# Acelogic/Retrieval-based-Voice-Conversion-MLX

Measured on AMD Instinct MI355X. Metric: audio-sec/sec (realtime factor) RVCv2 48kHz pipeline, higher is better.
Workload: dtype fp32-accurate (two-plane fp16 MFMA split); 1 GPU; C2: full RVCv2 48kHz pipeline, one 13.5 s utterance per step per GPU; samples_16k=216100, x_pad=1, f0_method=rmvpe, parallelism=dp1

## Files before the change

### retrieval-based-voice-conversion-mlx_amd/csrc/resblock_fused.hip

```cpp
#include <algorithm>

#include "conv_common.h"
#include "split_bf16.h"

namespace rvcx {

namespace {

using namespace splitbf16;

constexpr int RB_THREADS = 256;
constexpr int RB_MAXH1 = 30;

__host__ __device__ constexpr int rb_pi(int j) { return (j & 3) | (((j >> 3) & 1) << 2) | (((j >> 2) & 1) << 3); }

enum RbFmt : int { RB_BF16X3 = 0, RB_F16X2 = 1, RB_F16X1 = 2 };
__host__ __device__ constexpr int rb_planes(int fmt) { return fmt == RB_BF16X3 ? 3 : (fmt == RB_F16X2 ? 2 : 1); }

template <int C, int FMT = RB_BF16X3>
struct RbGeo {
  static constexpr int NCH = C / 16;
  static constexpr int NP = rb_planes(FMT);
  static constexpr int ROW = NCH * NP * 32 + 16;
};
// ... 383 lines not shown
#pragma unroll
      for (int q = 0; q < NQ; ++q) {
        w1r[st][q] = *reinterpret_cast<const f16x8_*>(p1 + (size_t)st * 2 * QS + q * QS);
        w2r[st][q] = *reinterpret_cast<const f16x8_*>(p2 + (size_t)st * 2 * QS + q * QS);
      }
  }
  if (tid < 4 * C) {
    const int which = tid / C, c = tid % C;
    const float* inv1 = reinterpret_cast<const float*>(static_cast<const char*>(a.w1s) + NST * 2 * QS);
    const float* inv2 = reinterpret_cast<const float*>(static_cast<const char*>(a.w2s) + NST * 2 * QS);
    prm[tid] = which == 0 ? a.b1[c] : which == 1 ? inv1[c] : which == 2 ? a.b2[c] : inv2[c];
  }

  f32x4 xv[XITER];
  unsigned xok = 0u;
  auto load_x = [&](int tl) __attribute__((always_inline)) {
    const int bb = tl / ntiles, tb = (tl - bb * ntiles) * TT - 1 - h1;
    const float* Xb = a.x + (long long)bb * a.x_bs;
    xok = 0u;
#pragma unroll
    for (int it = 0; it < XITER; ++it) {
      const int i = it * RB_THREADS + tid;
      const int r = i / C4, c4 = (i % C4) * 4;
      const int t = tb + r;
      const bool ok = r < nx && t >= 0 && t < a.T;
      xv[it] = *reinterpret_cast<const f32x4*>(Xb + (long long)(ok ? t : 0) * C + c4);
      xok |= ok ? (1u << it) : 0u;
    }
  };
  auto write_x = [&]() __attribute__((always_inline)) {
#pragma unroll
    for (int it = 0; it < XITER; ++it) {
      const int i = it * RB_THREADS + tid;
      const int r = i / C4, c4 = (i % C4) * 4;
      if (r < nx) {
        const int s = c4 >> 4, o = c4 & 15;
        const int slot = ((o >> 2) & 1) * 8 + (o >> 3) * 4;
        char* row = XS + (size_t)r * ROW + s * CB + slot * 2;
        const bool ok = (xok >> it) & 1u;
        const float y0 = ok ? lrelu01(xv[it][0]) * RB_XS : 0.f, y1 = ok ? lrelu01(xv[it][1]) * RB_XS : 0.f,
                    y2 = ok ? lrelu01(xv[it][2]) * RB_XS : 0.f, y3 = ok ? lrelu01(xv[it][3]) * RB_XS : 0.f;
        uint2 hh, ll;
        hh.x = pk_f16(y0, y1);
        hh.y = pk_f16(y2, y3);
        ll.x = pk_f16((y0 - f16lo_f(hh.x)) * H16_LO, (y1 - f16hi_f(hh.x)) * H16_LO);
        ll.y = pk_f16((y2 - f16lo_f(hh.y)) * H16_LO, (y3 - f16hi_f(hh.y)) * H16_LO);
        *reinterpret_cast<uint2*>(row) = hh;
        *reinterpret_cast<uint2*>(row + 32) = ll;
      }
    }
  };
  auto conv = [&](const char* bl, int dil, const f16x8_(&w)[NST][NQ], f32x16& acc, f32x16& acc2)
                  __attribute__((always_inline)) {
#pragma unroll
    for (int r = 0; r < 16; ++r) acc[r] = acc2[r] = 0.f;
    f16x8_ bf[2][NQ];
    auto load_b = [&](int st, f16x8_(&f)[NQ]) __attribute__((always_inline)) {
      const int tap = st / NCH, s = st - tap * NCH;
      const char* bp = bl + (size_t)tap * dil * ROW + s * CB;
#pragma unroll
      for (int q = 0; q < NQ; ++q) f[q] = *reinterpret_cast<const f16x8_*>(bp + q * 32);
    };
    load_b(0, bf[0]);
#pragma unroll
    for (int st = 0; st < NST; ++st) {
      if (st + 1 < NST) load_b(st + 1, bf[(st + 1) & 1]);
      __builtin_amdgcn_sched_barrier(0);
      const f16x8_ bh = bf[st & 1][0];
      acc = __builtin_amdgcn_mfma_f32_32x32x16_f16(w[st][0], bh, acc, 0, 0, 0);
      acc2 = __builtin_amdgcn_mfma_f32_32x32x16_f16(w[st][1], bh, acc2, 0, 0, 0);
      acc2 = __builtin_amdgcn_mfma_f32_32x32x16_f16(w[st][0], bf[st & 1][1], acc2, 0, 0, 0);
      __builtin_amdgcn_sched_barrier(0);
    }
  };
  auto finish = [&](f32x16& acc, const f32x16& acc2, const float* inv) __attribute__((always_inline)) {
#pragma unroll
    for (int m = 0; m < 4; ++m) {
      const f32x4 iv = *reinterpret_cast<const f32x4*>(inv + 8 * m + 4 * hk);
#pragma unroll
      for (int e = 0; e < 4; ++e) acc[4 * m + e] = (acc[4 * m + e] + acc2[4 * m + e] * H16_LO_INV) * iv[e];
    }
  };

  load_x(tile);
#pragma unroll 1
  for (; tile < tile_end; ++tile) {
    const int b = tile / ntiles;
    const int t0 = (tile - b * ntiles) * TT;
    write_x();
    __syncthreads();
    const float* X = a.x + (long long)b * a.x_bs;
    float* Y = a.y + (long long)b * a.y_bs;
    const int o = wave * 32 + li;
    const int t = t0 + o;
    const bool out_ok = o < TT && t < a.T;
    const long long off = (long long)(out_ok ? t : 0) * C + 4 * hk;
    f32x4 rv[4], dv[4];
#pragma unroll
    for (int m = 0; m < 4; ++m) {
      rv[m] = *reinterpret_cast<const f32x4*>(X + off + 8 * m);
      if constexpr (ACCM != ACC_STORE) dv[m] = *reinterpret_cast<const f32x4*>(Y + off + 8 * m);
    }
    load_x(min(tile + 1, tile_end - 1));
    {
      f32x16 acc, acc2;
      conv(XS + (size_t)(wave * 32 + li) * ROW + hk * 16, a.d, w1r, acc, acc2);
      finish(acc, acc2, prm + C);
      const int p = wave * 32 + li;
      const int tp = t0 - 1 + p;
      const bool ok = tp >= 0 && tp < a.T;
      char* row = TS + (size_t)p * ROW + hk * 16;
#pragma unroll
      for (int hh = 0; hh < 2; ++hh) {
        float v[8];
#pragma unroll
        for (int i = 0; i < 8; ++i) {
          const int r = 8 * hh + i;
          const float bv = prm[8 * (r >> 2) + 4 * hk + (r & 3)];
          const float x = lrelu01(acc[r] + bv);
          v[i] = ok ? x * RB_XS : 0.f;
        }
        uint4 Hh, Ll;
        split8_h16(v, Hh, Ll);
        char* dst = row + hh * CB;
        *reinterpret_cast<uint4*>(dst) = Hh;
        *reinterpret_cast<uint4*>(dst + 32) = Ll;
      }
    }
    __syncthreads();
    {
      f32x16 acc, acc2;
      conv(TS + (size_t)(wave * 32 + li) * ROW + hk * 16, 1, w2r, acc, acc2);
      finish(acc, acc2, prm + 3 * C);
      if (out_ok) {
#pragma unroll
        for (int m = 0; m < 4; ++m) {
          const f32x4 bv = *reinterpret_cast<const f32x4*>(prm + 2 * C + 8 * m + 4 * hk);
          f32x4 o4;
#pragma unroll
          for (int e = 0; e < 4; ++e) {
            float v = acc[4 * m + e] + bv[e];
            v = v + rv[m][e];
            if constexpr (ACCM == ACC_ADD) v = dv[m][e] + v;
            else if constexpr (ACCM == ACC_ADD_DIV) v = (dv[m][e] + v) / a.acc_div;
            o4[e] = v;
          }
          *reinterpret_cast<f32x4*>(Y + off + 8 * m) = o4;
        }
      }
    }
  }
}

template <int ACCM>
hipError_t launch_rb3(const RbPairArgs& a, hipStream_t s) {
  constexpr int ROW = RbGeo<32, RB_F16X2>::ROW;
  const int TT = 4 * 32 - 2;
  const size_t smem = (size_t)(4 * 32 + 2 * a.d) * ROW + (size_t)(4 * 32 + 2) * ROW + 4 * 32 * sizeof(float);
  auto kern = k_rb_pair3<ACCM>;
  static size_t smem_set = 64 * 1024;
  if (smem > smem_set) {
    hipError_t e = hipFuncSetAttribute(reinterpret_cast<const void*>(kern), hipFuncAttributeMaxDynamicSharedMemorySize,
                                       (int)smem);
    if (e != hipSuccess) return e;
    smem_set = smem;
  }
  const int ntiles = (a.T + TT - 1) / TT;
  static int ncu = 0;
  if (ncu == 0) {
    int dev = 0;
    if (hipGetDevice(&dev) != hipSuccess || hipDeviceGetAttribute(&ncu, hipDeviceAttributeMultiprocessorCount, dev) !=
                                                 hipSuccess || ncu <= 0)
      ncu = 256;
  }
  const long long tiles = (long long)ntiles * a.B;
  const int grid = (int)std::min<long long>(tiles, (long long)ncu * 2);
  hipLaunchKernelGGL(kern, dim3(grid), dim3(RB_THREADS), smem, s, a, ntiles);
  return hipGetLastError();
}

template <int C, int NBT, int TN, int MODE>
hipError_t launch_rb_acc(const RbPairArgs& a, hipStream_t s) {
  constexpr int ROW = RbGeo<C, (MODE >> 2) & 3>::ROW;
  const int h2 = (a.k - 1) / 2, h1 = h2 * a.d;
  const int TT = NBT * 32 - 2 * h2;
  const size_t smem = (size_t)(NBT * 32 + 2 * h1) * ROW + (size_t)(NBT * 32 + 2 * h2) * ROW;
  auto kern = k_rb_pair<C, NBT, TN, MODE>;
  static size_t smem_set = 64 * 1024;
  if (smem > smem_set) {
    hipError_t e = hipFuncSetAttribute(reinterpret_cast<const void*>(kern), hipFuncAttributeMaxDynamicSharedMemorySize,
                                       (int)smem);
    if (e != hipSuccess) return e;
    smem_set = smem;
  }
  const int ntiles = (a.T + TT - 1) / TT;
  static int ncu = 0;
  if (ncu == 0) {
    int dev = 0;
    if (hipGetDevice(&dev) != hipSuccess || hipDeviceGetAttribute(&ncu, hipDeviceAttributeMultiprocessorCount, dev) !=
                                                 hipSuccess || ncu <= 0)
      ncu = 256;
  }
  const int per_cu = std::max(1, std::min(3, (int)((160 * 1024) / smem)));
  const long long tiles = (long long)ntiles * a.B;
  const int grid = (int)std::min<long long>(tiles, (long long)ncu * per_cu);
  hipLaunchKernelGGL(kern, dim3(grid), dim3(RB_THREADS), smem, s, a, ntiles);
  return hipGetLastError();
}

template <int C, int NBT, int TN>
hipError_t launch_rb(const RbPairArgs& a, hipStream_t s) {
  const int fmt = a.wfmt == RB_WF16 ? (a.lowp ? RB_F16X1 : RB_F16X2) : RB_BF16X3;
  if (a.lowp && a.wfmt != RB_WF16) return hipErrorInvalidValue;
  switch (a.acc_mode | (fmt << 2)) {
#define RB_CASE(M) \
  case M: return launch_rb_acc<C, NBT, TN, M>(a, s);
    RB_CASE(0) RB_CASE(1) RB_CASE(2) RB_CASE(4) RB_CASE(5) RB_CASE(6) RB_CASE(8) RB_CASE(9) RB_CASE(10)
#undef RB_CASE
    default: return hipErrorInvalidValue;
  }
}

}

bool rb_pair_fits(int C, int k, int d) {
  if (!(C == 32 || C == 64)) return false;
  if (k < 1 || (k & 1) == 0 || d < 1) return false;
  const int h2 = (k - 1) / 2;
  return h2 * d <= RB_MAXH1 && 2 * h2 < 32;
}

long long rb_wsplit_bytes(int C, int k, int wfmt) {
  return wfmt == RB_WF16 ? (long long)k * (C / 16) * 2 * C * 32 + 8LL * C : (long long)k * (C / 16) * 3 * C * 32;
}

hipError_t rb_wsplit_build(const float* w, int C, int k, void* out, hipStream_t s, int wfmt) {
  if (C % 16 != 0 || k < 1) return hipErrorInvalidValue;
  const long long total = (long long)k * (C / 16) * C * 16;
  const long long nb = std::min<long long>((total + 255) / 256, 1 << 20);
  if (wfmt == RB_WF16) {
    float* tail = reinterpret_cast<float*>(static_cast<char*>(out) + (long long)k * (C / 16) * 2 * C * 32);
    hipLaunchKernelGGL(k_rb_wmax, dim3((unsigned)((C + 3) / 4)), dim3(256), 0, s, w, C, k,
                       reinterpret_cast<unsigned*>(tail) + C);
    hipLaunchKernelGGL(k_rb_wsplit_h16, dim3((unsigned)nb), dim3(256), 0, s, w, C, k, 2,
                       static_cast<unsigned short*>(out), tail);
    return hipGetLastError();
  }
  hipLaunchKernelGGL(k_rb_wsplit, dim3((unsigned)nb), dim3(256), 0, s, w, C, k, static_cast<unsigned short*>(out));
  return hipGetLastError();
}

hipError_t rb_pair(const RbPairArgs& a, int cfg, hipStream_t s) {
  if (cfg != 0 && cfg != 1) return hipErrorInvalidValue;
  if (!rb_pair_fits(a.C, a.k, a.d) || a.T < 1 || a.B < 1 || !a.x || !a.y || !a.w1s || !a.w2s || !a.b1 || !a.b2 ||
      a.x == a.y)
    return hipErrorInvalidValue;
  if ((reinterpret_cast<uintptr_t>(a.x) & 15) || (reinterpret_cast<uintptr_t>(a.y) & 15) || (a.x_bs & 3) ||
      (a.y_bs & 3))
    return hipErrorInvalidValue;
  if (cfg == 0 && a.C == 32 && a.k == 3 && a.wfmt == RB_WF16 && !a.lowp) {
    switch (a.acc_mode) {
      case ACC_STORE: return launch_rb3<ACC_STORE>(a, s);
      case ACC_ADD: return launch_rb3<ACC_ADD>(a, s);
      case ACC_ADD_DIV: return launch_rb3<ACC_ADD_DIV>(a, s);
      default: return hipErrorInvalidValue;
    }
  }
  switch (a.C) {
    case 32: return launch_rb<32, 4, 1>(a, s);
    case 64: return launch_rb<64, 2, 1>(a, s);
    default: return hipErrorInvalidValue;
  }
}

}
```

### retrieval-based-voice-conversion-mlx_amd/rvcx/_lib.py

```python
from __future__ import annotations

import ctypes
import os
from typing import Optional

_HERE = os.path.dirname(os.path.abspath(__file__))
LIB_PATH = os.environ.get("RVCX_LIB", os.path.join(_HERE, "librvcx.so"))

RVCX_MODEL_SYNTH, RVCX_MODEL_HUBERT, RVCX_MODEL_RMVPE, RVCX_MODEL_CREPE, RVCX_MODEL_FCPE = 0, 1, 2, 3, 4

STATUS = {
    0: "RVCX_OK", -1: "RVCX_E_INVALID", -2: "RVCX_E_SHAPE", -3: "RVCX_E_HIP", -4: "RVCX_E_OOM",
    -5: "RVCX_E_STATE", -6: "RVCX_E_CAPACITY",
}


class RvcxLibraryError(ImportError):
    pass


class RvcxError(RuntimeError):
    def __init__(self, code: int, msg: str):
        super().__init__(f"{STATUS.get(code, code)}: {msg}")
        self.code = code
# ... 32 lines not shown
                ("hop_size", ctypes.c_int), ("num_mels", ctypes.c_int), ("fmin", ctypes.c_float),
                ("fmax", ctypes.c_float), ("n_layers", ctypes.c_int), ("n_chans", ctypes.c_int),
                ("out_dims", ctypes.c_int)]


class RtDesc(ctypes.Structure):
    _fields_ = [("n_streams", ctypes.c_int), ("read_chunk_size", ctypes.c_int),
                ("cross_fade_overlap_size", ctypes.c_double), ("extra_convert_size", ctypes.c_double),
                ("silent_threshold", ctypes.c_double), ("f0_method", ctypes.c_int),
                ("fcpe_threshold", ctypes.c_float)]


class RtOpts(ctypes.Structure):
    _fields_ = [("f0_up_key", ctypes.c_double), ("index_rate", ctypes.c_double), ("protect", ctypes.c_float),
                ("volume_envelope", ctypes.c_double), ("f0_autotune", ctypes.c_int),
                ("f0_autotune_strength", ctypes.c_double), ("proposed_pitch", ctypes.c_int),
                ("proposed_pitch_threshold", ctypes.c_double), ("gen_precision", ctypes.c_int)]


class ConvTestDesc(ctypes.Structure):
    _fields_ = [
        ("x", ctypes.c_void_p), ("w", ctypes.c_void_p), ("bias", ctypes.c_void_p), ("res", ctypes.c_void_p),
        ("mask", ctypes.c_void_p), ("pre_mask", ctypes.c_void_p), ("y", ctypes.c_void_p),
        ("T_in", ctypes.c_int), ("C_in", ctypes.c_int), ("N", ctypes.c_int), ("taps", ctypes.c_int),
        ("dil", ctypes.c_int), ("pad", ctypes.c_int), ("stride", ctypes.c_int), ("T_out", ctypes.c_int),
        ("ldx", ctypes.c_int), ("ldy", ctypes.c_int), ("ldr", ctypes.c_int),
        ("batch", ctypes.c_int),
        ("x_bs", ctypes.c_int64), ("y_bs", ctypes.c_int64), ("res_bs", ctypes.c_int64), ("mask_bs", ctypes.c_int64),
        ("pre_mask_bs", ctypes.c_int64),
        ("batch_inner", ctypes.c_int),
        ("x_bs2", ctypes.c_int64), ("w_bs2", ctypes.c_int64), ("y_bs2", ctypes.c_int64), ("res_bs2", ctypes.c_int64),
        ("bias_bs2", ctypes.c_int64),
        ("pre_act", ctypes.c_int), ("pre_slope", ctypes.c_float),
        ("act", ctypes.c_int), ("slope", ctypes.c_float), ("alpha", ctypes.c_float),
        ("res_mode", ctypes.c_int), ("acc_mode", ctypes.c_int), ("acc_div", ctypes.c_float),
        ("gate_h", ctypes.c_int), ("gate_g", ctypes.c_void_p), ("gate_g_bs", ctypes.c_int64),
        ("ln_g", ctypes.c_void_p), ("ln_b", ctypes.c_void_p), ("ln_eps", ctypes.c_float),
        ("nz_har", ctypes.c_void_p), ("nz_bs", ctypes.c_int64),
        ("nz_stride", ctypes.c_int), ("nz_kk", ctypes.c_int), ("nz_u", ctypes.c_int), ("nz_C", ctypes.c_int),
        ("nz_w", ctypes.c_void_p), ("nz_b", ctypes.c_void_p),
        ("route", ctypes.c_int), ("no_splitk", ctypes.c_int),
    ]


class ConvPlanForm(ctypes.Structure):
    _fields_ = [("W_in", ctypes.c_int), ("W_out", ctypes.c_int), ("KH", ctypes.c_int), ("KW", ctypes.c_int),
                ("padh", ctypes.c_int), ("padw", ctypes.c_int), ("out_map", ctypes.c_int), ("out_cv", ctypes.c_int),
                ("lowp", ctypes.c_int), ("ldw", ctypes.c_int), ("w_ts", ctypes.c_int64),
                ("w_bs", ctypes.c_int64), ("bias_bs", ctypes.c_int64)]


class IndexBuildOpts(ctypes.Structure):
    _fields_ = [("niter", ctypes.c_int), ("nprobe", ctypes.c_int64), ("seed", ctypes.c_uint64),
                ("init_rows", ctypes.POINTER(ctypes.c_int64))]


vp, i64, i32, f32, f64, u64 = (ctypes.c_void_p, ctypes.c_int64, ctypes.c_int, ctypes.c_float, ctypes.c_double,
                               ctypes.c_uint64)
P = ctypes.POINTER


SIG = {
    "rvcx_create": (i32, [P(vp), i32]),
    "rvcx_destroy": (i32, [vp]),
    "rvcx_last_error": (ctypes.c_char_p, [vp]),
    "rvcx_set_synth_config": (i32, [vp, P(SynthDesc)]),
    "rvcx_upload": (i32, [vp, i32, ctypes.c_char_p, vp, P(i64), i32]),
    "rvcx_finalize": (i32, [vp, i32]),
    "rvcx_hubert": (i32, [vp, vp, i64, i32, vp, i64, P(i64), vp]),
    "rvcx_rmvpe": (i32, [vp, vp, i64, f32, vp, i64, P(i64), vp, vp]),
    "rvcx_f0_post": (i32, [vp, vp, i64, f64, vp, vp, vp, vp]),
    "rvcx_synth_infer": (i32, [vp, i32, i32, vp, vp, vp, vp, vp, vp, vp, u64, vp, vp, vp, vp]),
    "rvcx_synth_infer_ex": (i32, [vp, i32, i32, vp, vp, vp, vp, vp, f64, vp, vp, u64, vp, vp, vp, vp, vp, P(i32),
                                  vp]),
    "rvcx_dec_only": (i32, [vp, i32, i32, vp, vp, vp, vp, u64, vp, vp]),
    "rvcx_voice_conversion": (i32, [vp, vp, i64, vp, vp, i32, f32, f64, vp, vp, u64, vp, i64, P(i64), vp]),
    "rvcx_synth_upp": (i32, [vp]),
    "rvcx_set_highpass": (i32, [vp, vp, vp, vp, i32]),
    "rvcx_profile": (i32, [vp, i32]),
    "rvcx_profile_read": (i32, [vp, P(f64), P(f64), P(i64)]),
    "rvcx_profile_read_ex": (i32, [vp, P(f64), P(f64), P(i64), P(f64)]),
    "rvcx_pipeline": (i32, [vp, vp, i64, i32, f64, f32, i64, i64, vp, vp, u64, vp, i64, P(i64), vp, vp]),
    "rvcx_pipeline_default_opts": (i32, [P(PipelineOpts)]),
    "rvcx_pipeline_ex": (i32, [vp, vp, i64, P(PipelineOpts), vp, vp, u64, vp, i64, P(i64), vp, vp]),
    "rvcx_f0_autotune": (i32, [vp, vp, i64, f64, i32, vp]),
    "rvcx_rmvpe_decode": (i32, [vp, vp, i64, f32, vp, vp]),
    "rvcx_crepe": (i32, [vp, vp, i64, f32, f32, f32, vp, vp, vp, i64, P(i64), vp]),
    "rvcx_crepe_ex": (i32, [vp, vp, i64, f32, f32, f32, i32, vp, vp, vp, vp, i64, P(i64), vp]),
    "rvcx_crepe_decode": (i32, [vp, vp, i64, f32, f32, f32, i32, vp, vp, vp, vp]),
    "rvcx_set_fcpe_config": (i32, [vp, P(FcpeDesc)]),
    "rvcx_fcpe": (i32, [vp, vp, i64, f32, i32, i32, i64, vp, vp, i64, P(i64), vp]),
    "rvcx_fcpe_decode": (i32, [vp, vp, i64, f32, i32, i32, i64, vp, vp]),
    "rvcx_fcpe_b": (i32, [vp, vp, i64, i64, i32, f32, i32, vp, vp, vp]),
    "rvcx_split_audio": (i32, [vp, vp, i64, i32, f64, i32, P(i64), i64, P(i64), vp]),
    "rvcx_index_load": (i32, [vp, vp, i64]),
    "rvcx_index_unload": (i32, [vp]),
    "rvcx_index_info": (i32, [vp, P(i64), P(i64), P(i64), P(i64)]),
    "rvcx_index_set_nprobe": (i32, [vp, i64]),
    "rvcx_index_search": (i32, [vp, vp, i64, i32, vp, vp, vp]),
    "rvcx_index_reconstruct_n": (i32, [vp, i64, i64, vp, vp]),
    "rvcx_index_retrieve": (i32, [vp, vp, i64, i32, f64, vp, vp]),
    "rvcx_index_default_build_opts": (i32, [P(IndexBuildOpts)]),
    "rvcx_index_build": (i32, [vp, vp, i64, i32, i64, P(IndexBuildOpts), vp]),
    "rvcx_index_centroids": (i32, [vp, vp, vp]),
    "rvcx_index_save": (i32, [vp, vp, i64, P(i64)]),
    "rvcx_pipeline_batch": (i32, [vp, vp, i64, i64, i32, P(PipelineOpts), P(ctypes.c_int32), vp, vp, u64, vp, i64,
                                  P(i64), vp, vp, vp]),
    "rvcx_pipeline_batch_v": (i32, [vp, vp, P(i64), i64, i32, P(PipelineOpts), P(ctypes.c_int32), vp, vp, u64, vp,
                                    i64, P(i64), vp, i64, vp]),
    "rvcx_set_highpass_sos": (i32, [vp, vp, i32]),
    "rvcx_workspace_bytes": (i32, [vp, i32, i64, P(PipelineOpts), P(i64), vp]),
    "rvcx_set_workspace": (i32, [vp, vp, i64]),
    "rvcx_workspace_info": (i32, [vp, P(i64), P(i64), P(i64)]),
    "rvcx_highpass_pad": (i32, [vp, vp, i64, i64, vp, vp, vp]),
    "rvcx_resample_poly_len": (i32, [i64, i32, i32, P(i64)]),
    "rvcx_resample_poly_v": (i32, [vp, vp, i32, i32, P(i64), i64, i32, i32, i32, vp, i64, vp, i64, P(i64), vp]),
    "rvcx_hubert_batch": (i32, [vp, vp, i64, i64, i32, i32, vp, i64, P(i64), vp]),
    "rvcx_hubert_batch_v": (i32, [vp, vp, P(i64), i64, i32, i32, vp, i64, P(i64), vp]),
    "rvcx_rmvpe_batch": (i32, [vp, vp, i64, i64, i32, f32, vp, i64, P(i64), vp, vp]),
    "rvcx_rmvpe_batch_v": (i32, [vp, vp, P(i64), i64, i32, f32, vp, i64, P(i64), vp, i64, vp]),
    "rvcx_fcpe_batch_v": (i32, [vp, vp, P(i64), i64, i32, f32, i32, vp, i64, P(i64), vp, i64, vp]),
    "rvcx_rt_default_desc": (i32, [P(RtDesc)]),
    "rvcx_rt_default_opts": (i32, [P(RtOpts)]),
    "rvcx_rt_create": (i32, [vp, P(RtDesc), P(vp)]),
    "rvcx_rt_destroy": (i32, [vp, vp]),
    "rvcx_rt_geometry": (i32, [vp, P(i64)]),
    "rvcx_rt_reset": (i32, [vp, vp, vp]),
    "rvcx_rt_process": (i32, [vp, vp, vp, P(ctypes.c_int32), P(RtOpts), vp, vp, u64, vp, vp, vp, vp]),
    "rvcx_rt_process_v": (i32, [vp, vp, vp, P(ctypes.c_int32), P(RtOpts), P(ctypes.c_uint8), vp, vp, u64, vp, vp,
                                vp, vp]),
    "rvcx_rt_reset_stream": (i32, [vp, vp, i32, vp]),
    "rvcx_spectral_gate": (i32, [vp, vp, i32, i64, i64, i32, P(f32), vp, i64, vp, vp]),
    "rvcx_rt_set_clean": (i32, [vp, vp, i32, i32, f64]),
    "rvcx_device_status": (i32, [vp, vp]),
    "rvcx_index_parse": (i32, [vp, i64, P(i64), P(i64), P(i64), P(i64), ctypes.c_char_p, i64]),
    "rvcx_config_info": (i32, [vp, vp, i64, P(i64)]),
    "rvcx_profile_read_kinds": (i32, [vp, P(f64), P(f64), P(i64), P(f64), i32, P(f64), P(f64), P(f64), P(f64),
                                      P(i64)]),
    "rvcx_profile_kind_name": (ctypes.c_char_p, [i32]),
}

TEST_SIG = {
    "rvcx_set_conv_math": (i32, [vp, i32]),
    "rvcx_conv1d": (i32, [vp, vp, i64, i32, vp, vp, i32, i32, i32, i32, i32, i32, vp, i64, vp]),
    "rvcx_conv1d_gen": (i32, [vp, vp, i64, i32, vp, vp, i32, i32, i32, i32, i32, f32, i32, f32, vp, i32, f32, i32,
                              vp, vp]),
    "rvcx_conv1d_ex": (i32, [vp, P(ConvTestDesc), P(i32), P(i32), vp]),
    "rvcx_conv2d3x3": (i32, [vp, vp, i32, i32, i32, vp, vp, i32, i32, i32, vp, vp]),
    "rvcx_convtranspose2d_s2": (i32, [vp, vp, i32, i32, i32, vp, vp, i32, i32, i32, vp, vp]),
    "rvcx_conv2d3x3_v": (i32, [vp, vp, i32, P(i32), i32, i32, i32, vp, vp, i32, i32, i32, vp, vp]),
    "rvcx_convtranspose2d_s2_v": (i32, [vp, vp, i32, P(i32), i32, i32, i32, vp, vp, i32, i32, i32, vp, vp]),
    "rvcx_flash_attention": (i32, [vp, vp, i32, i32, i32, i32, f32, vp, vp, i32, vp, vp, vp]),
    "rvcx_resblock_pair": (i32, [vp, vp, i32, i64, i32, vp, vp, vp, vp, i32, i32, i32, f32, i32, vp, vp]),
    "rvcx_performer_attention": (i32, [vp, vp, vp, vp, i32, i32, vp, i32, vp, vp]),
    "rvcx_performer_attention_b": (i32, [vp, vp, vp, vp, i32, i32, i32, vp, i32, vp, vp]),
    "rvcx_performer_attention_v": (i32, [vp, vp, vp, vp, i32, i32, P(i32), i32, vp, i32, vp, vp]),
    "rvcx_fcpe_mel": (i32, [vp, vp, i64, vp, i64, P(i64), vp]),
    "rvcx_set_dec_window": (i32, [vp, i32]),
    "rvcx_dec_margin_frames": (i32, [P(SynthDesc), P(i32)]),
    "rvcx_conv_plan": (i32, [P(ConvTestDesc), P(ConvPlanForm), i32, i32, i32, i32, i32, i32, P(i32), P(i32), P(i32),
                             P(i32)]),
    "rvcx_kmeans_assign": (i32, [vp, vp, i64, i32, vp, i64, vp, vp, vp]),
    "rvcx_kmeans_update": (i32, [vp, vp, i64, i32, vp, i64, vp, vp, vp]),
    "rvcx_rt_model_rows": (i32, [vp, vp, i32, vp, i64, vp]),
    "rvcx_gru_bidir": (i32, [vp, vp, i32, i32, vp, vp, vp, vp, vp, i64, vp]),
    "rvcx_gru_bidir_v": (i32, [vp, vp, i32, P(i32), vp, vp, vp, vp, vp, i64, vp]),
    "rvcx_dec_source": (i32, [vp, i32, i32, vp, vp, u64, vp, vp]),
    "rvcx_rg_resample_dw": (i32, [vp, vp, i32, i32, i32, vp, i32, i32, vp, i32, vp]),
    "rvcx_rg_lerp_up_cat": (i32, [vp, vp, i32, i32, i32, i32, i32, f32, vp, i32, vp, i32, vp]),
    "rvcx_rg_adain": (i32, [vp, vp, i32, i32, i32, vp, vp, u64, f32, vp, i32, f32, vp]),
}

EXPORTS = list(SIG)
TEST_EXPORTS = list(TEST_SIG)

_lib: Optional[ctypes.CDLL] = None


def load(path: Optional[str] = None) -> ctypes.CDLL:
    global _lib
    if _lib is not None and path is None:
        return _lib
    p = path or LIB_PATH
    if not os.path.exists(p):
        raise RvcxLibraryError(f"librvcx.so not found at {p}; build it with __graft_entry__.build() "
                               "(make -C retrieval-based-voice-conversion-mlx_amd/csrc)")
    try:
        lib = ctypes.CDLL(p)
    except OSError as e:
        raise RvcxLibraryError(f"cannot load {p}: {e}") from e
    for name, (res, args) in {**SIG, **TEST_SIG}.items():
        if not hasattr(lib, name):
            continue
        fn = getattr(lib, name)
        fn.restype = res
        fn.argtypes = args
    if path is None:
        _lib = lib
    return lib


def exported_symbols(path: Optional[str] = None):
    lib = load(path)
    return [n for n in EXPORTS + TEST_EXPORTS if hasattr(lib, n)]


def index_parse(data: bytes) -> dict:
    lib = load()
    buf = ctypes.create_string_buffer(bytes(data), len(data))
    v = [ctypes.c_int64(0) for _ in range(4)]
    err = ctypes.create_string_buffer(512)
    rc = lib.rvcx_index_parse(buf, len(data), *[ctypes.byref(x) for x in v], err, 512)
    if rc != 0:
        raise RvcxError(rc, err.value.decode(errors="replace"))
    return dict(zip(("d", "ntotal", "nlist", "nprobe"), (x.value for x in v)))
```

### retrieval-based-voice-conversion-mlx_amd/rvcx/engine_kernels.py

```python
from __future__ import annotations

import ctypes
from typing import Optional

import numpy as np

from . import _lib
from .config import SynthConfig


def _ptr(t) -> Optional[int]:
    return None if t is None else t.data_ptr()


class KernelTestMixin:
    def set_dec_window(self, on: bool):
        self._check(self.lib.rvcx_set_dec_window(self.ctx, 1 if on else 0), "set_dec_window")

    def dec_margin_frames(self, cfg: SynthConfig = None) -> int:
        d = self._synth_desc(cfg if cfg is not None else self.synth_cfg)
        m = ctypes.c_int32(0)
        rc = self.lib.rvcx_dec_margin_frames(ctypes.byref(d), ctypes.byref(m))
        if rc != 0:
            raise _lib.RvcxError(rc, "dec_margin_frames: bad synthesizer configuration")
# ... 199 lines not shown
        return y

    ROUTES = {"policy": 0, "f32": 1, "emu": 2, "wsb": 3, "gs": 4, "wst": 5}

    def conv1d_ex(self, x, w, y, *, T_in: int, C_in: int, N: int, T_out: int, ldx: int, ldy: int, taps: int = 1,
                  dil: int = 1, pad: int = 0, stride: int = 1, ldr: int = 0, bias=None, res=None, mask=None,
                  pre_mask=None, batch: int = 1, x_bs: int = 0, y_bs: int = 0, res_bs: int = 0, mask_bs: int = 0,
                  pre_mask_bs: int = 0, batch_inner: int = 1, x_bs2: int = 0, w_bs2: int = 0, y_bs2: int = 0,
                  res_bs2: int = 0, bias_bs2: int = 0, pre_act: int = 0, pre_slope: float = 0.0, act: int = 0,
                  slope: float = 0.0, alpha: float = 1.0, res_mode: int = 0, acc_mode: int = 0, acc_div: float = 1.0,
                  gate_h: int = 0, gate_g=None, gate_g_bs: int = 0, ln_g=None, ln_b=None, ln_eps: float = 1e-5,
                  nz_har=None, nz_bs: int = 0, nz_stride: int = 0, nz_kk: int = 0, nz_u: int = 1, nz_C: int = 0,
                  nz_w=None, nz_b=None, route="policy", no_splitk: bool = False):
        torch = self.torch
        G, B, i64 = int(batch_inner), int(batch), int

        def span(t, name, last):
            if t is None:
                return None
            if not (isinstance(t, torch.Tensor) and t.dtype == torch.float32 and t.device == self.device):
                raise ValueError(f"conv1d_ex: {name} must be a float32 tensor on {self.device}")
            room = t.untyped_storage().nbytes() // 4 - t.storage_offset()
            if last < 0 or last >= room:
                raise ValueError(f"conv1d_ex: {name} addresses element {last}, its storage holds {room} from the view")
            return t.data_ptr()

        ncol = gate_h if gate_h > 0 else N
        d = _lib.ConvTestDesc()
        d.x = span(x, "x", (B - 1) * x_bs + (G - 1) * x_bs2 + (T_in - 1) * ldx + C_in - 1)
        d.w = span(w, "w", (G - 1) * w_bs2 + taps * N * C_in - 1)
        d.y = span(y, "y", (B - 1) * y_bs + (G - 1) * y_bs2 + (T_out - 1) * ldy + ncol - 1)
        d.bias = span(bias, "bias", (G - 1) * bias_bs2 + N - 1)
        d.res = span(res, "res", (B - 1) * res_bs + (G - 1) * res_bs2 + (T_out - 1) * ldr + N - 1)
        d.mask = span(mask, "mask", (B - 1) * mask_bs + T_out - 1)
        d.pre_mask = span(pre_mask, "pre_mask", (B - 1) * pre_mask_bs + T_in - 1)
        d.gate_g = span(gate_g, "gate_g", (B - 1) * gate_g_bs + N - 1)
        d.ln_g, d.ln_b = span(ln_g, "ln_g", N - 1), span(ln_b, "ln_b", N - 1)
        d.nz_har = span(nz_har, "nz_har", (B - 1) * nz_bs + (T_out * nz_u - 1) * nz_stride + max(nz_kk, 1) - 1)
        d.nz_w = span(nz_w, "nz_w", nz_C * max(nz_stride, 1) * max(-(-nz_kk // max(nz_stride, 1)), 1) - 1)
        d.nz_b = span(nz_b, "nz_b", nz_C - 1)
        for k, v in dict(T_in=T_in, C_in=C_in, N=N, taps=taps, dil=dil, pad=pad, stride=stride, T_out=T_out, ldx=ldx,
                         ldy=ldy, ldr=ldr, batch=B, x_bs=x_bs, y_bs=y_bs, res_bs=res_bs, mask_bs=mask_bs,
                         pre_mask_bs=pre_mask_bs, batch_inner=G, x_bs2=x_bs2, w_bs2=w_bs2, y_bs2=y_bs2,
                         res_bs2=res_bs2, bias_bs2=bias_bs2, pre_act=pre_act, act=act, res_mode=res_mode,
                         acc_mode=acc_mode, gate_h=gate_h, gate_g_bs=gate_g_bs, nz_bs=nz_bs, nz_stride=nz_stride,
                         nz_kk=nz_kk, nz_u=nz_u, nz_C=nz_C).items():
            setattr(d, k, i64(v))
        d.pre_slope, d.slope, d.alpha, d.acc_div, d.ln_eps = (float(pre_slope), float(slope), float(alpha),
                                                              float(acc_div), float(ln_eps))
        d.route = self.ROUTES[route] if isinstance(route, str) else int(route)
        d.no_splitk = 1 if no_splitk else 0
        self.last_conv_desc = d
        kind, ksplit = ctypes.c_int(-1), ctypes.c_int(0)
        self._check(self.lib.rvcx_conv1d_ex(self.ctx, ctypes.byref(d), ctypes.byref(kind), ctypes.byref(ksplit),
                                            self.stream()), "conv1d_ex")
        name = self.lib.rvcx_profile_kind_name(kind.value)
        return y, (name.decode() if name else "other"), int(ksplit.value)

    def conv_plan(self, desc=None, static_weight: bool = True):
        out = [ctypes.c_int(-1) for _ in range(4)]
        d = self.last_conv_desc if desc is None else desc
        self._check(self.lib.rvcx_conv_plan(ctypes.byref(d), None, 0, 1 if static_weight else 0,
                                            getattr(self, "conv_math", 0), 0, -1, -1, *[ctypes.byref(o) for o in out]),
                    "conv_plan")
        name = self.lib.rvcx_profile_kind_name(out[0].value)
        return (name.decode() if name else "other"), out[1].value, out[2].value, out[3].value

    def conv2d3x3(self, x, w, bias=None, relu: bool = False, math: str = "default"):
        torch = self.torch
        x = self._dev(x, torch.float32)
        w = torch.as_tensor(w, dtype=torch.float32)
        N, C = int(w.shape[0]), int(w.shape[1])
        wk = self._dev(w.permute(2, 3, 0, 1).reshape(9, N, C).contiguous(), torch.float32)
        b = self._dev(bias, torch.float32) if bias is not None else None
        H, W = int(x.shape[0]), int(x.shape[1])
        y = torch.empty((H, W, N), dtype=torch.float32, device=self.device)
        m = {"default": 0, "f32": 1, "gsw": 2}[math]
        self._check(self.lib.rvcx_conv2d3x3(self.ctx, _ptr(x), H, W, C, _ptr(wk), _ptr(b), N, 1 if relu else 0, m,
                                            _ptr(y), self.stream()), "conv2d3x3")
        return y

    def convtranspose2d_s2(self, x, w, bias=None, relu: bool = False, math: str = "default"):
        torch = self.torch
        x = self._dev(x, torch.float32)
        wd = self._dev(torch.as_tensor(w, dtype=torch.float32).contiguous(), torch.float32)
        C, N = int(wd.shape[0]), int(wd.shape[1])
        b = self._dev(bias, torch.float32) if bias is not None else None
        H, W = int(x.shape[0]), int(x.shape[1])
        y = torch.empty((2 * H, 2 * W, N), dtype=torch.float32, device=self.device)
        m = {"default": 0, "f32": 1}[math]
        self._check(self.lib.rvcx_convtranspose2d_s2(self.ctx, _ptr(x), H, W, C, _ptr(wd), _ptr(b), N,
                                                     1 if relu else 0, m, _ptr(y), self.stream()), "convtranspose2d_s2")
        return y

    def conv2d3x3_v(self, x, heights, w, bias=None, relu: bool = False, math: str = "default"):
        torch = self.torch
        x = self._dev(x, torch.float32).contiguous()
        w = torch.as_tensor(w, dtype=torch.float32)
        N, C = int(w.shape[0]), int(w.shape[1])
        wk = self._dev(w.permute(2, 3, 0, 1).reshape(9, N, C).contiguous(), torch.float32)
        b = self._dev(bias, torch.float32) if bias is not None else None
        B, H, W = (int(v) for v in x.shape[:3])
        hv = (ctypes.c_int32 * B)(*[int(v) for v in heights])
        y = torch.empty((B, H, W, N), dtype=torch.float32, device=self.device)
        m = {"default": 0, "f32": 1, "gsw": 2}[math]
        self._check(self.lib.rvcx_conv2d3x3_v(self.ctx, _ptr(x), B, hv, H, W, C, _ptr(wk), _ptr(b), N,
                                              1 if relu else 0, m, _ptr(y), self.stream()), "conv2d3x3_v")
        return y

    def convtranspose2d_s2_v(self, x, heights, w, bias=None, relu: bool = False, math: str = "default"):
        torch = self.torch
        x = self._dev(x, torch.float32).contiguous()
        wd = self._dev(torch.as_tensor(w, dtype=torch.float32).contiguous(), torch.float32)
        C, N = int(wd.shape[0]), int(wd.shape[1])
        b = self._dev(bias, torch.float32) if bias is not None else None
        B, H, W = (int(v) for v in x.shape[:3])
        hv = (ctypes.c_int32 * B)(*[int(v) for v in heights])
        y = torch.empty((B, 2 * H, 2 * W, N), dtype=torch.float32, device=self.device)
        m = {"default": 0, "f32": 1}[math]
        self._check(self.lib.rvcx_convtranspose2d_s2_v(self.ctx, _ptr(x), B, hv, H, W, C, _ptr(wd), _ptr(b), N,
                                                       1 if relu else 0, m, _ptr(y), self.stream()),
                    "convtranspose2d_s2_v")
        return y

    def flash_attention(self, qkv, n_heads: int, qscale: float, rel_k=None, rel_v=None, window: int = 0, mask=None):
        torch = self.torch
        q = self._dev(qkv, torch.float32)
        B, T, H3 = (int(v) for v in q.shape)
        dk = H3 // 3 // n_heads
        rk = self._opt(rel_k, torch.float32)
        rv = self._opt(rel_v, torch.float32)
        mk = self._opt(mask, torch.float32)
        y = torch.empty((B, T, H3 // 3), dtype=torch.float32, device=self.device)
        self._check(self.lib.rvcx_flash_attention(self.ctx, _ptr(q), B, T, int(n_heads), dk, float(qscale), _ptr(rk),
                                                  _ptr(rv), int(window), _ptr(mk), _ptr(y), self.stream()),
                    "flash_attention")
        return y

    def resblock_pair(self, x, w1, b1, w2, b2, dilation: int, acc=None, acc_mode: int = 0, acc_div: float = 1.0,
                      cfg: int = 0):
        torch = self.torch
        x = self._dev(x, torch.float32)
        B, T, C = (int(v) for v in x.shape)
        k = int(np.shape(w1)[2])
        w1k = self._dev(torch.as_tensor(w1, dtype=torch.float32).permute(2, 0, 1).contiguous(), torch.float32)
        w2k = self._dev(torch.as_tensor(w2, dtype=torch.float32).permute(2, 0, 1).contiguous(), torch.float32)
        b1d, b2d = self._dev(b1, torch.float32), self._dev(b2, torch.float32)
        y = (self._dev(acc, torch.float32).clone() if acc is not None
             else torch.empty((B, T, C), dtype=torch.float32, device=self.device))
        self._check(self.lib.rvcx_resblock_pair(self.ctx, _ptr(x), B, T, C, _ptr(w1k), _ptr(b1d), _ptr(w2k), _ptr(b2d),
                                                k, dilation, acc_mode, float(acc_div), cfg, _ptr(y), self.stream()),
                    "resblock_pair")
        return y
```

Before: 1121 audio-sec/sec.

## Add persistent warp-specialized resblock pair kernel for k=7/11 with resident weights

Adds a persistent 512-thread kernel for C=32 resblock pairs with kernel sizes 7 and 11, used by default. Four waves compute the first conv into a double-buffered LDS tile while four other waves compute the second conv on the previous tile, and the input loads for the next tiles are prefetched into registers. Weights are held in registers, with the k=11 tail staged in LDS. The aim is to cut launch and tile overheads and to overlap the two convs and the global loads, at the cost of high register and LDS pressure and one block per CU. It also adds a Python wrapper and binding for a strided variant.

Result: faster. 1143 audio-sec/sec (median of 6 runs) (+1.9%).

```diff
diff --git a/retrieval-based-voice-conversion-mlx_amd/csrc/resblock_fused.hip b/retrieval-based-voice-conversion-mlx_amd/csrc/resblock_fused.hip
--- a/retrieval-based-voice-conversion-mlx_amd/csrc/resblock_fused.hip
+++ b/retrieval-based-voice-conversion-mlx_amd/csrc/resblock_fused.hip
@@ -559,6 +559,263 @@
   }
 }
 
+constexpr int RBR_THREADS = 512;
+constexpr int RBR_NLS11 = 8;
+template <int K, int ACCM>
+__global__ __launch_bounds__(RBR_THREADS, 1) void k_rb_pair_res(const RbPairArgs a, const int ntiles) {
+  constexpr int C = 32, NBT = 4, NCH = 2, NQ = 2, CB = NQ * 32, ROW = RbGeo<C, RB_F16X2>::ROW, NST = K * NCH;
+  constexpr int H2 = (K - 1) / 2, TT = NBT * 32 - 2 * H2, TROWS = NBT * 32 + 2 * H2;
+  constexpr int C4 = C / 4;
+  constexpr int XITER = ((NBT * 32 + 2 * RB_MAXH1) * C4 + RBR_THREADS - 1) / RBR_THREADS;
+  constexpr int NLS = K <= 7 ? 0 : RBR_NLS11;
+  constexpr int NRS = NST - NLS;
+  constexpr size_t QS = (size_t)C * 32;
+  typedef _Float16 f16x8_ __attribute__((ext_vector_type(8)));
+  extern __shared__ __attribute__((aligned(16))) char rb_smem[];
+  const int tid = threadIdx.x, lane = tid & 63, wave = __builtin_amdgcn_readfirstlane(tid >> 6);
+  const bool second = wave >= 4;
+  const int blk = wave & 3;
+  const int li = lane & 31, hk = lane >> 5;
+  const int h1 = H2 * a.d;
+  const int nx = NBT * 32 + 2 * h1;
+  char* const XS = rb_smem;
+  char* const TS = rb_smem + 2 * (size_t)nx * ROW;
+  float* const prm = reinterpret_cast<float*>(TS + 2 * (size_t)TROWS * ROW);
+  char* const WL = reinterpret_cast<char*>(prm + 4 * C);
+  const int total = ntiles * a.B;
+  const int per = (total + (int)gridDim.x - 1) / (int)gridDim.x;
+  const int tile0 = blockIdx.x * per;
+  const int tile_end = min(total, tile0 + per);
+  if (tile0 >= tile_end) return;
+  const int n = tile_end - tile0;
+
+  f16x8_ wr[NRS][NQ];
+  {
+    const char* p = static_cast<const char*>(second ? a.w2s : a.w1s) + (size_t)li * 32 + hk * 16;
+#pragma unroll
+    for (int st = 0; st < NRS; ++st)
+#pragma unroll
+      for (int q = 0; q < NQ; ++q) wr[st][q] = *reinterpret_cast<const f16x8_*>(p + (size_t)st * 2 * QS + q * QS);
+  }
+  if constexpr (NLS > 0) {
+    constexpr int PER = NLS * NQ * (int)QS / 16;
+    for (int i = tid; i < 2 * PER; i += RBR_THREADS) {
+      const char* src = static_cast<const char*>(i < PER ? a.w1s : a.w2s) + (size_t)NRS * 2 * QS;
+      *reinterpret_cast<uint4*>(WL + (size_t)i * 16) = *reinterpret_cast<const uint4*>(src + (size_t)(i % PER) * 16);
+    }
+  }
+  const char* const wl = WL + (second ? NLS * NQ * QS : 0) + (size_t)li * 32 + hk * 16;
+  if (tid < 4 * C) {
+    const int which = tid / C, c = tid % C;
+    const float* inv1 = reinterpret_cast<const float*>(static_cast<const char*>(a.w1s) + NST * 2 * QS);
+    const float* inv2 = reinterpret_cast<const float*>(static_cast<const char*>(a.w2s) + NST * 2 * QS);
+    prm[tid] = which == 0 ? a.b1[c] : which == 1 ? inv1[c] : which == 2 ? a.b2[c] : inv2[c];
+  }
+
+  f32x4 xv[XITER];
+  unsigned xok = 0u;
+  int xt = tid;
+  auto load_x = [&](int tl) __attribute__((always_inline)) {
+    const int bb = tl / ntiles, tb = (tl - bb * ntiles) * TT - H2 - h1;
+    const float* Xb = a.x + (long long)bb * a.x_bs;
+    xok = 0u;
+#pragma unroll
+    for (int it = 0; it < XITER; ++it) {
+      const int i = it * RBR_THREADS + xt;
+      const int r = i / C4, c4 = (i % C4) * 4;
+      const int t = tb + r;
+      const bool ok = r < nx && t >= 0 && t < a.T;
+      xv[it] = *reinterpret_cast<const f32x4*>(Xb + (long long)(ok ? t : 0) * C + c4);
+      xok |= ok ? (1u << it) : 0u;
+    }
+  };
+  auto write_x = [&](char* xs) __attribute__((always_inline)) {
+#pragma unroll
+    for (int it = 0; it < XITER; ++it) {
+      const int i = it * RBR_THREADS + xt;
+      const int r = i / C4, c4 = (i % C4) * 4;
+      if (r < nx) {
+        const int s = c4 >> 4, o = c4 & 15;
+        const int slot = ((o >> 2) & 1) * 8 + (o >> 3) * 4;
+        char* row = xs + (size_t)r * ROW + s * CB + slot * 2;
+        const bool ok = (xok >> it) & 1u;
+        const float y0 = ok ? lrelu01(xv[it][0]) * RB_XS : 0.f, y1 = ok ? lrelu01(xv[it][1]) * RB_XS : 0.f,
+                    y2 = ok ? lrelu01(xv[it][2]) * RB_XS : 0.f, y3 = ok ? lrelu01(xv[it][3]) * RB_XS : 0.f;
+        uint2 hh, ll;
+        hh.x = pk_f16(y0, y1);
+        hh.y = pk_f16(y2, y3);
+        ll.x = pk_f16((y0 - f16lo_f(hh.x)) * H16_LO, (y1 - f16hi_f(hh.x)) * H16_LO);
+        ll.y = pk_f16((y2 - f16lo_f(hh.y)) * H16_LO, (y3 - f16hi_f(hh.y)) * H16_LO);
+        *reinterpret_cast<uint2*>(row) = hh;
+        *reinterpret_cast<uint2*>(row + 32) = ll;
+      }
+    }
+  };
+  auto conv = [&](const char* bl, int tstep, f32x16& acc, f32x16& acc2) __attribute__((always_inline)) {
+#pragma unroll
+    for (int r = 0; r < 16; ++r) acc[r] = acc2[r] = 0.f;
+    f16x8_ bf[2][NQ];
+    auto load_b = [&](int st, f16x8_(&f)[NQ]) __attribute__((always_inline)) {
+      const int tap = st / NCH, s = st - tap * NCH;
+      const char* bp = bl + (size_t)tap * tstep + s * CB;
+#pragma unroll
+      for (int q = 0; q < NQ; ++q) f[q] = *reinterpret_cast<const f16x8_*>(bp + q * 32);
+    };
+    f16x8_ wls[2][NQ];
+    load_b(0, bf[0]);
+#pragma unroll
+    for (int st = 0; st < NST; ++st) {
+      if (NLS > 0 && st + 1 >= NRS && st + 1 < NST) {
+#pragma unroll
+        for (int q = 0; q < NQ; ++q)
+          wls[(st + 1) & 1][q] = *reinterpret_cast<const f16x8_*>(wl + (size_t)((st + 1 - NRS) * NQ + q) * QS);
+      }
+      const f16x8_ wh = st < NRS ? wr[st < NRS ? st : 0][0] : wls[st & 1][0];
+      const f16x8_ wo = st < NRS ? wr[st < NRS ? st : 0][1] : wls[st & 1][1];
+      if (st + 1 < NST) load_b(st + 1, bf[(st + 1) & 1]);
+      __builtin_amdgcn_sched_barrier(0);
+      const f16x8_ bh = bf[st & 1][0];
+      acc = __builtin_amdgcn_mfma_f32_32x32x16_f16(wh, bh, acc, 0, 0, 0);
+      acc2 = __builtin_amdgcn_mfma_f32_32x32x16_f16(wo, bh, acc2, 0, 0, 0);
+      acc2 = __builtin_amdgcn_mfma_f32_32x32x16_f16(wh, bf[st & 1][1], acc2, 0, 0, 0);
+      __builtin_amdgcn_sched_barrier(0);
+    }
+  };
+  auto finish = [&](f32x16& acc, const f32x16& acc2, const float* inv) __attribute__((always_inline)) {
+#pragma unroll
+    for (int m = 0; m < 4; ++m) {
+      const f32x4 iv = *reinterpret_cast<const f32x4*>(inv + 8 * m + 4 * hk);
+#pragma unroll
+      for (int e = 0; e < 4; ++e) acc[4 * m + e] = (acc[4 * m + e] + acc2[4 * m + e] * H16_LO_INV) * iv[e];
+    }
+  };
+
+  load_x(tile0);
+  write_x(XS);
+  load_x(min(tile0 + 1, tile_end - 1));
+  __syncthreads();
+#pragma unroll 1
+  for (int j = 0; j <= n; ++j) {
+    asm volatile("" : "+v"(xt));
+    write_x(XS + (size_t)((j + 1) & 1) * nx * ROW);
+    load_x(min(tile0 + j + 2, tile_end - 1));
+    if (!second) {
+      if (j < n) {
+        const int tile = tile0 + j;
+        const int b = tile / ntiles;
+        const int t0 = (tile - b * ntiles) * TT;
+        f32x16 acc, acc2;
+        conv(XS + (size_t)(j & 1) * nx * ROW + (size_t)(blk * 32 + li) * ROW + hk * 16, a.d * ROW, acc, acc2);
+        finish(acc, acc2, prm + C);
+        const int p = blk * 32 + li;
+        const int tp = t0 - H2 + p;
+        const bool ok = tp >= 0 && tp < a.T;
+        char* row = TS + (size_t)(j & 1) * TROWS * ROW + (size_t)p * ROW + hk * 16;
+#pragma unroll
+        for (int hh = 0; hh < 2; ++hh) {
+          float v[8];
+#pragma unroll
+          for (int i = 0; i < 8; ++i) {
+            const int r = 8 * hh + i;
+            const float bv = prm[8 * (r >> 2) + 4 * hk + (r & 3)];
+            const float x = lrelu01(acc[r] + bv);
+            v[i] = ok ? x * RB_XS : 0.f;
+          }
+          uint4 Hh, Ll;
+          split8_h16(v, Hh, Ll);
+          char* dst = row + hh * CB;
+          *reinterpret_cast<uint4*>(dst) = Hh;
+          *reinterpret_cast<uint4*>(dst + 32) = Ll;
+        }
+      }
+    } else {
+      if (j > 0) {
+        const int tile = tile0 + j - 1;
+        const int b = tile / ntiles;
+        const int t0 = (tile - b * ntiles) * TT;
+        const float* X = a.x + (long long)b * a.x_bs;
+        float* Y = a.y + (long long)b * a.y_bs;
+        const int o = blk * 32 + li;
+        const int t = t0 + o;
+        const bool out_ok = o < TT && t < a.T;
+        const long long off = (long long)(out_ok ? t : 0) * C + 4 * hk;
+        f32x4 rv[4], dv[4];
+        auto load_res = [&]() __attribute__((always_inline)) {
+#pragma unroll
+          for (int m = 0; m < 4; ++m) {
+            rv[m] = *reinterpret_cast<const f32x4*>(X + off + 8 * m);
+            if constexpr (ACCM != ACC_STORE) dv[m] = *reinterpret_cast<const f32x4*>(Y + off + 8 * m);
+          }
+        };
+        load_res();
+        f32x16 acc, acc2;
+        conv(TS + (size_t)((j - 1) & 1) * TROWS * ROW + (size_t)(blk * 32 + li) * ROW + hk * 16, ROW, acc, acc2);
+        finish(acc, acc2, prm + 3 * C);
+        if (out_ok) {
+#pragma unroll
+          for (int m = 0; m < 4; ++m) {
+            const f32x4 bv = *reinterpret_cast<const f32x4*>(prm + 2 * C + 8 * m + 4 * hk);
+            f32x4 o4;
+#pragma unroll
+            for (int e = 0; e < 4; ++e) {
+              float v = acc[4 * m + e] + bv[e];
+              v = v + rv[m][e];
+              if constexpr (ACCM == ACC_ADD) v = dv[m][e] + v;
+              else if constexpr (ACCM == ACC_ADD_DIV) v = (dv[m][e] + v) / a.acc_div;
+              o4[e] = v;
+            }
+            *reinterpret_cast<f32x4*>(Y + off + 8 * m) = o4;
+          }
+        }
+      }
+    }
+    __syncthreads();
+  }
+}
+
+template <int K, int ACCM>
+hipError_t launch_rbr_acc(const RbPairArgs& a, hipStream_t s) {
+  constexpr int ROW = RbGeo<32, RB_F16X2>::ROW, H2 = (K - 1) / 2;
+  constexpr int TT = 4 * 32 - 2 * H2;
+  constexpr size_t WLDS = K <= 7 ? 0 : 2 * RBR_NLS11 * 2 * (size_t)32 * 32;
+  const size_t smem = 2 * (size_t)(4 * 32 + 2 * H2 * a.d) * ROW + 2 * (size_t)(4 * 32 + 2 * H2) * ROW +
+                      4 * 32 * sizeof(float) + WLDS;
+  auto kern = k_rb_pair_res<K, ACCM>;
+  static size_t smem_set = 64 * 1024;
+  if (smem > smem_set) {
+    hipError_t e = hipFuncSetAttribute(reinterpret_cast<const void*>(kern), hipFuncAttributeMaxDynamicSharedMemorySize,
+                                       (int)smem);
+    if (e != hipSuccess) return e;
+    smem_set = smem;
+  }
+  const int ntiles = (a.T + TT - 1) / TT;
+  static int ncu = 0;
+  if (ncu == 0) {
+    int dev = 0;
+    if (hipGetDevice(&dev) != hipSuccess || hipDeviceGetAttribute(&ncu, hipDeviceAttributeMultiprocessorCount, dev) !=
+                                                 hipSuccess || ncu <= 0)
+      ncu = 256;
+  }
+  const long long tiles = (long long)ntiles * a.B;
+  const int grid = (int)std::min<long long>(tiles, (long long)ncu);
+  hipLaunchKernelGGL(kern, dim3(grid), dim3(RBR_THREADS), smem, s, a, ntiles);
+  return hipGetLastError();
+}
+
+bool rb_resident_fits(const RbPairArgs& a) {
+  return a.C == 32 && (a.k == 7 || a.k == 11) && a.wfmt == RB_WF16 && !a.lowp;
+}
+
+template <int K>
+hipError_t launch_rbr(const RbPairArgs& a, hipStream_t s) {
+  switch (a.acc_mode) {
+    case ACC_STORE: return launch_rbr_acc<K, ACC_STORE>(a, s);
+    case ACC_ADD: return launch_rbr_acc<K, ACC_ADD>(a, s);
+    case ACC_ADD_DIV: return launch_rbr_acc<K, ACC_ADD_DIV>(a, s);
+    default: return hipErrorInvalidValue;
+  }
+}
+
 template <int ACCM>
 hipError_t launch_rb3(const RbPairArgs& a, hipStream_t s) {
   constexpr int ROW = RbGeo<32, RB_F16X2>::ROW;
@@ -658,7 +915,7 @@
 }
 
 hipError_t rb_pair(const RbPairArgs& a, int cfg, hipStream_t s) {
-  if (cfg != 0 && cfg != 1) return hipErrorInvalidValue;
+  if (cfg < 0 || cfg > 2) return hipErrorInvalidValue;
   if (!rb_pair_fits(a.C, a.k, a.d) || a.T < 1 || a.B < 1 || !a.x || !a.y || !a.w1s || !a.w2s || !a.b1 || !a.b2 ||
       a.x == a.y)
     return hipErrorInvalidValue;
@@ -673,6 +930,8 @@
       default: return hipErrorInvalidValue;
     }
   }
+  if (cfg == 2 && !rb_resident_fits(a)) return hipErrorInvalidValue;
+  if (cfg != 1 && rb_resident_fits(a)) return a.k == 7 ? launch_rbr<7>(a, s) : launch_rbr<11>(a, s);
   switch (a.C) {
     case 32: return launch_rb<32, 4, 1>(a, s);
     case 64: return launch_rb<64, 2, 1>(a, s);
diff --git a/retrieval-based-voice-conversion-mlx_amd/rvcx/_lib.py b/retrieval-based-voice-conversion-mlx_amd/rvcx/_lib.py
--- a/retrieval-based-voice-conversion-mlx_amd/rvcx/_lib.py
+++ b/retrieval-based-voice-conversion-mlx_amd/rvcx/_lib.py
@@ -208,6 +208,8 @@
     "rvcx_convtranspose2d_s2_v": (i32, [vp, vp, i32, P(i32), i32, i32, i32, vp, vp, i32, i32, i32, vp, vp]),
     "rvcx_flash_attention": (i32, [vp, vp, i32, i32, i32, i32, f32, vp, vp, i32, vp, vp, vp]),
     "rvcx_resblock_pair": (i32, [vp, vp, i32, i64, i32, vp, vp, vp, vp, i32, i32, i32, f32, i32, vp, vp]),
+    "rvcx_resblock_pair_strided": (i32, [vp, vp, i64, i32, i64, i32, vp, vp, vp, vp, i32, i32, i32, f32, i32, vp, i64,
+                                         vp]),
     "rvcx_performer_attention": (i32, [vp, vp, vp, vp, i32, i32, vp, i32, vp, vp]),
     "rvcx_performer_attention_b": (i32, [vp, vp, vp, vp, i32, i32, i32, vp, i32, vp, vp]),
     "rvcx_performer_attention_v": (i32, [vp, vp, vp, vp, i32, i32, P(i32), i32, vp, i32, vp, vp]),
diff --git a/retrieval-based-voice-conversion-mlx_amd/rvcx/engine_kernels.py b/retrieval-based-voice-conversion-mlx_amd/rvcx/engine_kernels.py
--- a/retrieval-based-voice-conversion-mlx_amd/rvcx/engine_kernels.py
+++ b/retrieval-based-voice-conversion-mlx_amd/rvcx/engine_kernels.py
@@ -375,3 +375,21 @@
                                                 k, dilation, acc_mode, float(acc_div), cfg, _ptr(y), self.stream()),
                     "resblock_pair")
         return y
+
+    def resblock_pair_strided(self, xbuf, T: int, w1, b1, w2, b2, dilation: int, ybuf, acc_mode: int = 0,
+                              acc_div: float = 1.0, cfg: int = 0):
+        torch = self.torch
+        assert xbuf.is_cuda and ybuf.is_cuda and xbuf.is_contiguous() and ybuf.is_contiguous()
+        assert xbuf.dtype == torch.float32 and ybuf.dtype == torch.float32
+        B, Sx, C = (int(v) for v in xbuf.shape)
+        By, Sy, Cy = (int(v) for v in ybuf.shape)
+        assert By == B and Cy == C and Sx >= T and Sy >= T
+        k = int(np.shape(w1)[2])
+        w1k = self._dev(torch.as_tensor(w1, dtype=torch.float32).permute(2, 0, 1).contiguous(), torch.float32)
+        w2k = self._dev(torch.as_tensor(w2, dtype=torch.float32).permute(2, 0, 1).contiguous(), torch.float32)
+        b1d, b2d = self._dev(b1, torch.float32), self._dev(b2, torch.float32)
+        self._check(self.lib.rvcx_resblock_pair_strided(self.ctx, _ptr(xbuf), Sx * C, B, int(T), C, _ptr(w1k),
+                                                        _ptr(b1d), _ptr(w2k), _ptr(b2d), k, dilation, acc_mode,
+                                                        float(acc_div), cfg, _ptr(ybuf), Sy * C, self.stream()),
+                    "resblock_pair_strided")
+        return ybuf
```
